# jordi-adell/mcarray

Hardware: AMD Instinct MI355X
Metric: STFT frames/sec, 8-mic GCC-PHAT + SRP-PHAT(361) + delay-and-sum beamform @48kHz/1024-pt (higher is better)
Workload: dtype f32 (SRP operands adaptive); 1 GPU; BASELINE configs[2] geometry (8-mic ULA 0.04 m, 48 kHz, N=1024, hop 512, 361 angles, 1 source, no power floor), 8 arrays x 4096 frames per GPU per step; channel rows padded by 64 floats; arrays_per_gpu=8, frames_per_array=4096, srp_precision=adaptive, parallelism=arrays sharded over 1 GPU(s), all_gather of DOA bins+prob

## Files before the change

### mcarray_amd/csrc/api.hip

```cpp
#include "../../include/mcarray_hip.h"
#include "fft1024c.h"
#include "kernels.h"
#include "knobs.h"
#include "stage.h"

#include <chrono>
#include <cmath>
#include <cstdio>
#include <cstdlib>
#include <cstring>
#include <string>
#include <thread>
#include <vector>

using namespace mca;

namespace {

std::string g_create_error;

struct TimedEvent { int id; hipEvent_t a, b; };

}

// ... 1521 lines not shown
static int ensure_bf_table(mca_hip_ctx *c)
{
    if (!c->d_bftab && c->n2048) {
        HIP_TRY(c, hipMalloc((void **)&c->d_bftab, (size_t)(c->D + 1) * c->M * 1032 * sizeof(float2)));
        c->bf_pairs = c->M;
        const double unit = (double)c->cfg.sample_rate / (double)c->N / 346.1;
        hipLaunchKernelGGL(k_bf_table_2048, dim3(c->D + 1, c->M), dim3(256), 0, nullptr, c->d_bftab, c->d_grid, c->d_micx, c->M, unit);
        HIP_TRY(c, hipGetLastError());
        HIP_TRY(c, hipDeviceSynchronize());
        return MCA_HIP_OK;
    }
    if (c->d_bftab || !wave_beamformer_applies(c)) return MCA_HIP_OK;
    const int np = (c->M + 1) / 2;
    HIP_TRY(c, hipMalloc((void **)&c->d_bftab, (size_t)(c->D + 1) * np * 1024 * sizeof(float2)));
    c->bf_pairs = np;
    const double unit = (double)c->cfg.sample_rate / (double)FFT_N / 346.1;
    hipLaunchKernelGGL(k_bf_table, dim3(c->D + 1, np), dim3(256), 0, nullptr, c->d_bftab, c->d_grid, c->d_micx, c->M, np, unit);
    HIP_TRY(c, hipGetLastError());
    HIP_TRY(c, hipDeviceSynchronize());
    return MCA_HIP_OK;
}

static int separate_impl(mca_hip_ctx *c, const float *pcm, long long array_stride, long long mic_stride,
                         int n_arrays, int n_frames, const float *doa_rad, float *out_pcm, hipStream_t st, const int *doa_bin = nullptr)
{
    const size_t a0 = (size_t)c->a0;
    if (doa_bin && c->d_bftab && c->n2048 && (reinterpret_cast<uintptr_t>(out_pcm) & 7) == 0) {
        BeamformWaveArgs wa{};
        wa.pcm = pcm; wa.array_stride = array_stride; wa.mic_stride = mic_stride;
        wa.M = c->M; wa.n_pairs = c->M; wa.n_frames = n_frames; wa.S = c->S;
        wa.ft = 16;
        for (int ft = 2; ft <= 64; ++ft)
            if ((long long)n_arrays * c->S * ((n_frames + 4 * ft - 2) / (4 * ft - 1)) <= 2LL * c->n_cu) { wa.ft = ft; break; }
        wa.window = c->d_window; wa.doa_bin = doa_bin; wa.table = c->d_bftab; wa.out = out_pcm;
        wa.tail_in = c->d_tail[c->tail_cur] + a0 * c->S * c->H; wa.tail_out = c->d_tail[c->tail_cur ^ 1] + a0 * c->S * c->H;
        const int wgs = (n_frames + 4 * wa.ft - 2) / (4 * wa.ft - 1);
        const size_t smem_w = (size_t)(F1K_TWORDS + 4 * F1K_SCRATCH + 4 * 512) * sizeof(float2);
        time_begin(c, MCA_HIP_K_BEAMFORM, st);
        hipLaunchKernelGGL(k_beamform_wave_2048, dim3(wgs, n_arrays, c->S), dim3(256), smem_w, st, wa);
        time_end(c, st);
        HIP_TRY(c, hipGetLastError());
        return MCA_HIP_OK;
    }
    if (doa_bin && c->d_bftab && wave_beamformer_applies(c)) {
        BeamformWaveArgs wa{};
        wa.pcm = pcm; wa.array_stride = array_stride; wa.mic_stride = mic_stride;
        wa.M = c->M; wa.n_pairs = c->bf_pairs; wa.n_frames = n_frames; wa.S = c->S;
        wa.window = c->d_window; wa.doa_bin = doa_bin; wa.table = c->d_bftab; wa.out = out_pcm;
        wa.tail_in = c->d_tail[c->tail_cur] + a0 * c->S * c->H; wa.tail_out = c->d_tail[c->tail_cur ^ 1] + a0 * c->S * c->H;
        if (c->S >= 2 && c->M <= 8) {
            wa.ft = 16;
            while (wa.ft > 2 && (long long)n_arrays * ((n_frames + wa.ft - 1) / wa.ft) < 2048) wa.ft >>= 1;
            const int runs = (n_frames + wa.ft - 1) / wa.ft;
            const size_t smem_ms = (size_t)(F1K_TWORDS + 4 * F1K_SCRATCH) * sizeof(float2) + (size_t)4 * c->S * FFT_H * sizeof(float);
            const dim3 gms((runs + 3) / 4, n_arrays);
            time_begin(c, MCA_HIP_K_BEAMFORM, st);
#define BFMS(NPT)                                                                                                                   \
            do {                                                                                                                    \
                if (smem_ms > 64 * 1024) {                                                                                          \
                    HIP_TRY(c, hipFuncSetAttribute(reinterpret_cast<const void *>(&k_beamform_wave_ms<NPT, false>), hipFuncAttributeMaxDynamicSharedMemorySize, (int)smem_ms)); \
                    HIP_TRY(c, hipFuncSetAttribute(reinterpret_cast<const void *>(&k_beamform_wave_ms<NPT, true>), hipFuncAttributeMaxDynamicSharedMemorySize, (int)smem_ms));  \
                }                                                                                                                   \
                if (c->M & 1) hipLaunchKernelGGL((k_beamform_wave_ms<NPT, true>), gms, dim3(256), smem_ms, st, wa);                 \
                else hipLaunchKernelGGL((k_beamform_wave_ms<NPT, false>), gms, dim3(256), smem_ms, st, wa);                         \
            } while (0)
            if (c->bf_pairs == 1) {
                if (smem_ms > 64 * 1024) HIP_TRY(c, hipFuncSetAttribute(reinterpret_cast<const void *>(&k_beamform_wave_ms<1, false>), hipFuncAttributeMaxDynamicSharedMemorySize, (int)smem_ms));
                hipLaunchKernelGGL((k_beamform_wave_ms<1, false>), gms, dim3(256), smem_ms, st, wa);
            }
            else if (c->bf_pairs == 2) BFMS(2);
            else if (c->bf_pairs == 3) BFMS(3);
            else BFMS(4);
#undef BFMS
            time_end(c, st);
            HIP_TRY(c, hipGetLastError());
            return MCA_HIP_OK;
        }
        wa.ft = 2;
        while (wa.ft < 256 && (long long)n_arrays * c->S * ((n_frames + 4 * wa.ft - 2) / (4 * wa.ft - 1)) > 512) ++wa.ft;
        const int wgs = (n_frames + 4 * wa.ft - 2) / (4 * wa.ft - 1);
        const size_t smem = (size_t)(F1K_TWORDS + 4 * F1K_SCRATCH) * sizeof(float2) + 4 * FFT_H * sizeof(float);
        dim3 gb(wgs, n_arrays, c->S);
        if (c->S == 1 && (wgs & 1) == 0 && wa.ft >= 8 && (long long)wgs * n_arrays > (long long)c->n_cu * 3 / 2 && (long long)wgs * n_arrays <= 2LL * c->n_cu) {
            wa.skew = (3 * wa.ft + 8) / 16;
            if (wa.skew >= wa.ft) wa.skew = 0;
            else gb = dim3(n_arrays, wgs, c->S);
        }
        time_begin(c, MCA_HIP_K_BEAMFORM, st);
        if (c->M & 1) hipLaunchKernelGGL(k_beamform_wave<true>, gb, dim3(256), smem, st, wa);
        else hipLaunchKernelGGL(k_beamform_wave<false>, gb, dim3(256), smem, st, wa);
        time_end(c, st);
        HIP_TRY(c, hipGetLastError());
        return MCA_HIP_OK;
    }
    BeamformArgs ba{};
    ba.pcm = pcm; ba.array_stride = array_stride; ba.mic_stride = mic_stride;
    ba.M = c->M; ba.Mpad = c->M; ba.S = c->S; ba.n_frames = n_frames; ba.fs = c->cfg.sample_rate;
    ba.ft = 64;
    long long want_wgs = 512;
    if (c->generic) {
        const size_t smem_g = (size_t)(c->M + c->S) * (c->H + 1) * sizeof(float2) + (size_t)c->S * c->H * sizeof(float);
        const long long per_cu = std::max<long long>(1, std::min<long long>((160 * 1024) / (long long)smem_g, 2048 / gen_threads(c, true)));
        want_wgs = 256 * per_cu;
    }
    while (ba.ft > BF_NB && (long long)n_arrays * ((n_frames + ba.ft - 1) / ba.ft) < want_wgs) ba.ft >>= 1;
    ba.window = c->d_window; ba.mic_x = c->d_micx; ba.doa_rad = doa_rad; ba.out = out_pcm;
    ba.tail_in = c->d_tail[c->tail_cur] + a0 * c->S * c->H; ba.tail_out = c->d_tail[c->tail_cur ^ 1] + a0 * c->S * c->H;
    ba.N = c->N; ba.logH = c->logH; ba.tw = c->d_tw;
    if (c->n512) {
        const size_t smem = ((size_t)2 * 8 * 258 + 8 * FFT_SCRATCH + TW_WIN + (size_t)2 * c->S * c->M * 41) * sizeof(float2) + (size_t)2 * c->S * sizeof(double);
        ba.ft = 64;
        const long long per_cu = smem <= 80 * 1024 ? 2 : 1;
        while (ba.ft > 4 && (long long)n_arrays * ((n_frames + ba.ft - 1) / ba.ft) < 256 * per_cu) ba.ft >>= 1;
        HIP_TRY(c, hipFuncSetAttribute(reinterpret_cast<const void *>(k_beamform_512), hipFuncAttributeMaxDynamicSharedMemorySize, (int)smem));
        time_begin(c, MCA_HIP_K_BEAMFORM, st);
        hipLaunchKernelGGL(k_beamform_512, dim3((n_frames + ba.ft - 1) / ba.ft, n_arrays), dim3(512), smem, st, ba);
        time_end(c, st);
        HIP_TRY(c, hipGetLastError());
        return MCA_HIP_OK;
    }
    if (c->generic) {
        auto smem_for = [&](int s_pass) {
            return (size_t)(c->M + s_pass) * (c->H + 1) * sizeof(float2) + (size_t)s_pass * c->H * sizeof(float) + (size_t)(ba.ft + 1) * s_pass * sizeof(double) + 8;
        };
        int s_pass = c->S;
        while (s_pass > 1 && smem_for(s_pass) > 160 * 1024) --s_pass;
        const size_t smem = smem_for(s_pass);
        if (smem > 160 * 1024) return fail(c, MCA_HIP_ERR_UNSUPPORTED, "fft_size x n_mics exceeds the 160 KiB LDS of a CU");
        if (smem > 64 * 1024)
            HIP_TRY(c, hipFuncSetAttribute(reinterpret_cast<const void *>(k_beamform_gen), hipFuncAttributeMaxDynamicSharedMemorySize, (int)smem));
        time_begin(c, MCA_HIP_K_BEAMFORM, st);
        ba.S_all = c->S;
        for (int s0 = 0; s0 < c->S; s0 += s_pass) {
            ba.s0 = s0; ba.S = std::min(s_pass, c->S - s0);
// ... 740 lines not shown
```

### mcarray_amd/csrc/fft1024c.h

```cpp
#pragma once
#include "fft512.h"

namespace mca {

constexpr int F1K_ROW = 18;
constexpr int F1K_SCRATCH = 64 * F1K_ROW;
constexpr int F1K_TWORDS = 64 * F1K_ROW;

__device__ __forceinline__ void f1k_table_init(float2 *tab, int tid, int nthreads)
{
    for (int e = tid; e < 1024; e += nthreads) tab[(e >> 4) * F1K_ROW + (e & 15)] = twiddle(((e >> 4) * (e & 15)) & 1023, 1024, false);
}

__device__ __forceinline__ float2 csub_jb(float2 a, float2 b)
{
    v2f av = to_v2f(a), bv = to_v2f(b), r;
    asm("v_pk_fma_f32 %0, %2, 1.0, %1 op_sel:[1,0,0] op_sel_hi:[0,0,1] neg_hi:[1,0,0]" : "=v"(r) : "v"(av), "v"(bv));
    return from_v2f(r);
}
__device__ __forceinline__ float2 cadd_jb(float2 a, float2 b)
{
    v2f av = to_v2f(a), bv = to_v2f(b), r;
    asm("v_pk_fma_f32 %0, %2, 1.0, %1 op_sel:[1,0,0] op_sel_hi:[0,0,1] neg_lo:[1,0,0]" : "=v"(r) : "v"(av), "v"(bv));
    return from_v2f(r);
}
__device__ __forceinline__ float2 cscale(float2 a, float s)
{
    v2f av = to_v2f(a), sv = {s, s}, r;
    asm("v_pk_mul_f32 %0, %1, %2" : "=v"(r) : "v"(av), "v"(sv));
    return from_v2f(r);
}
__device__ __forceinline__ float2 cmul_mj(float2 a)
{
    v2f av = to_v2f(a), one = {1.f, 1.f}, r;
    asm("v_pk_mul_f32 %0, %1, %2 op_sel:[1,0] op_sel_hi:[0,1] neg_hi:[1,0]" : "=v"(r) : "v"(av), "v"(one));
    return from_v2f(r);
}
__device__ __forceinline__ float2 cmul_pj(float2 a)
{
    v2f av = to_v2f(a), one = {1.f, 1.f}, r;
    asm("v_pk_mul_f32 %0, %1, %2 op_sel:[1,0] op_sel_hi:[0,1] neg_lo:[1,0]" : "=v"(r) : "v"(av), "v"(one));
    return from_v2f(r);
}

template <bool INV>
__device__ __forceinline__ void bfly4(float2 &a0, float2 &a1, float2 &a2, float2 &a3)
{
    const float2 t0 = cadd(a0, a2), t1 = csub(a0, a2), t2 = cadd(a1, a3), t3 = csub(a1, a3);
    a0 = cadd(t0, t2);
    a2 = csub(t0, t2);
    if (!INV) { a1 = csub_jb(t1, t3); a3 = cadd_jb(t1, t3); }
    else { a1 = cadd_jb(t1, t3); a3 = csub_jb(t1, t3); }
}

__device__ __forceinline__ constexpr int dr16(int p) { return (p >> 2) + 4 * (p & 3); }

template <bool INV>
__device__ __forceinline__ void fft16(float2 (&v)[16])
{
    constexpr float R = 0.70710678118654752440f, C1 = 0.92387953251128675613f, S1 = 0.38268343236508977173f;
#pragma unroll
    for (int j = 0; j < 4; ++j) bfly4<INV>(v[j], v[j + 4], v[j + 8], v[j + 12]);
    const float2 w1 = make_float2(C1, -S1), w3 = make_float2(S1, -C1), w9 = make_float2(-C1, S1);
    if (!INV) {
        v[5] = cmul(v[5], w1);  v[9] = cscale(csub_jb(v[9], v[9]), R);   v[13] = cmul(v[13], w3);
        v[6] = cscale(csub_jb(v[6], v[6]), R);  v[10] = cmul_mj(v[10]);   v[14] = cscale(cadd_jb(v[14], v[14]), -R);
        v[7] = cmul(v[7], w3);  v[11] = cscale(cadd_jb(v[11], v[11]), -R); v[15] = cmul(v[15], w9);
    } else {
        v[5] = cmulc(v[5], w1); v[9] = cscale(cadd_jb(v[9], v[9]), R);   v[13] = cmulc(v[13], w3);
        v[6] = cscale(cadd_jb(v[6], v[6]), R);  v[10] = cmul_pj(v[10]);   v[14] = cscale(csub_jb(v[14], v[14]), -R);
        v[7] = cmulc(v[7], w3); v[11] = cscale(csub_jb(v[11], v[11]), -R); v[15] = cmulc(v[15], w9);
    }
#pragma unroll
    for (int q = 0; q < 4; ++q) bfly4<INV>(v[4 * q], v[4 * q + 1], v[4 * q + 2], v[4 * q + 3]);
}

__device__ __forceinline__ void lds_read16_b128(float2 (&v)[16], const float2 *p)
{
    typedef float v4f __attribute__((ext_vector_type(4)));
    v4f a[8];
    asm volatile(
        "ds_read_b128 %0, %8\n\tds_read_b128 %1, %8 offset:16\n\tds_read_b128 %2, %8 offset:32\n\tds_read_b128 %3, %8 offset:48\n\t"
        "ds_read_b128 %4, %8 offset:64\n\tds_read_b128 %5, %8 offset:80\n\tds_read_b128 %6, %8 offset:96\n\tds_read_b128 %7, %8 offset:112\n\t"
        "s_waitcnt lgkmcnt(0)"
        : "=&v"(a[0]), "=&v"(a[1]), "=&v"(a[2]), "=&v"(a[3]), "=&v"(a[4]), "=&v"(a[5]), "=&v"(a[6]), "=&v"(a[7])
        : "v"((unsigned)(uintptr_t)p)
        : "memory");
#pragma unroll
    for (int i = 0; i < 8; ++i) { v[2 * i] = make_float2(a[i].x, a[i].y); v[2 * i + 1] = make_float2(a[i].z, a[i].w); }
}

__device__ __forceinline__ void swap_rows32(float &a, float &b)
{
    const auto r = __builtin_amdgcn_permlane32_swap(__float_as_uint(a), __float_as_uint(b), false, false);
    a = __uint_as_float(r[0]); b = __uint_as_float(r[1]);
}
__device__ __forceinline__ void swap_rows16(float &a, float &b)
{
    const auto r = __builtin_amdgcn_permlane16_swap(__float_as_uint(a), __float_as_uint(b), false, false);
    a = __uint_as_float(r[0]); b = __uint_as_float(r[1]);
}
__device__ __forceinline__ void transpose_rows4(float2 &x0, float2 &x1, float2 &x2, float2 &x3)
{
    swap_rows32(x0.x, x2.x); swap_rows32(x0.y, x2.y); swap_rows32(x1.x, x3.x); swap_rows32(x1.y, x3.y);
    swap_rows16(x0.x, x1.x); swap_rows16(x0.y, x1.y); swap_rows16(x2.x, x3.x); swap_rows16(x2.y, x3.y);
}

struct F1kNoMid { __device__ __forceinline__ void operator()() const {} };

struct F1kLane {
    float2 wb[4];
    float2 t1[16];
    __device__ __forceinline__ void init(int lane)
    {
#pragma unroll
        for (int q = 1; q < 4; ++q) wb[q] = twiddle(((lane & 15) * q) & 63, 64, false);
    }
    __device__ __forceinline__ void load_t1(const float2 *tab, int lane)
    {
#pragma unroll
        for (int q = 0; q < 16; ++q) t1[q] = tab[lane * 18 + q];
    }
};

template <bool INV, int OPT = 3, typename Mid = F1kNoMid>
__device__ __forceinline__ void fft1024c(float2 (&v)[16], float2 *buf, int lane, const float2 *tab, const F1kLane &lc, Mid mid = Mid(), int row = -1)
{
    constexpr bool SCHED = OPT & 2, T1REG = OPT & 4;
    float2 tw[16];
    if (!T1REG) {
        lds_read16_b128(tw, tab + lane * F1K_ROW);
        if (SCHED) __builtin_amdgcn_sched_barrier(0);
    }
    fft16<INV>(v);
#pragma unroll
    for (int p = 1; p < 16; ++p) {
        const float2 w = T1REG ? lc.t1[dr16(p)] : tw[dr16(p)];
        v[p] = INV ? cmulc(v[p], w) : cmul(v[p], w);
    }
#pragma unroll
    for (int q = 0; q < 4; ++q) transpose_rows4(v[4 * q], v[4 * q + 1], v[4 * q + 2], v[4 * q + 3]);
#pragma unroll
    for (int q = 0; q < 4; ++q) bfly4<INV>(v[4 * q], v[4 * q + 1], v[4 * q + 2], v[4 * q + 3]);
    float2 *wr = buf + (lane >> 4) * (4 * F1K_ROW) + (lane & 15);
#pragma unroll
    for (int q = 0; q < 4; ++q)
#pragma unroll
        for (int kb = 0; kb < 4; ++kb) {
            if (kb != 0) v[4 * q + kb] = INV ? cmulc(v[4 * q + kb], lc.wb[kb]) : cmul(v[4 * q + kb], lc.wb[kb]);
            wr[(q + 16 * kb) * F1K_ROW] = v[4 * q + kb];
        }
    wave_lds_fence();
    mid();
    if (SCHED) __builtin_amdgcn_sched_barrier(0);
    lds_read16_b128(v, buf + (row < 0 ? lane : row) * F1K_ROW);
    wave_lds_fence();
    fft16<INV>(v);
}

}
```

### mcarray_amd/csrc/fft512.h

```cpp
#pragma once
#include <hip/hip_runtime.h>

namespace mca {

constexpr int FFT_N = 1024;
constexpr int FFT_H = 512;
constexpr int FFT_K = 513;
constexpr int FFT_SCRATCH = 576;
constexpr int FFT_ROW = 72;

typedef float v2f __attribute__((ext_vector_type(2)));
__device__ __forceinline__ v2f to_v2f(float2 a) { v2f r = {a.x, a.y}; return r; }
__device__ __forceinline__ float2 from_v2f(v2f a) { return make_float2(a.x, a.y); }

__device__ __forceinline__ float2 cmul(float2 a, float2 b)
{
    v2f av = to_v2f(a), bv = to_v2f(b), t, r;
    asm("v_pk_mul_f32 %0, %1, %2 op_sel:[1,0] op_sel_hi:[1,1]" : "=v"(t) : "v"(av), "v"(bv));
    asm("v_pk_fma_f32 %0, %1, %2, %3 op_sel:[0,0,1] op_sel_hi:[0,1,0] neg_lo:[0,0,1]" : "=v"(r) : "v"(av), "v"(bv), "v"(t));
    return from_v2f(r);
}
__device__ __forceinline__ float2 cmulc(float2 a, float2 b)
{
    v2f av = to_v2f(a), bv = to_v2f(b), t, r;
    asm("v_pk_mul_f32 %0, %1, %2 op_sel:[1,0] op_sel_hi:[1,1]" : "=v"(t) : "v"(bv), "v"(av));
    asm("v_pk_fma_f32 %0, %1, %2, %3 op_sel:[0,0,1] op_sel_hi:[1,0,0] neg_hi:[0,0,1]" : "=v"(r) : "v"(av), "v"(bv), "v"(t));
    return from_v2f(r);
}
__device__ __forceinline__ float2 cmac(float2 acc, float2 a, float2 b)
{
    v2f av = to_v2f(a), bv = to_v2f(b), cv = to_v2f(acc), u, r;
    asm("v_pk_fma_f32 %0, %1, %2, %3 op_sel:[1,0,1] op_sel_hi:[1,1,0] neg_hi:[1,0,0]" : "=v"(u) : "v"(bv), "v"(av), "v"(cv));
    asm("v_pk_fma_f32 %0, %1, %2, %3 op_sel:[0,0,1] op_sel_hi:[1,0,0]" : "=v"(r) : "v"(av), "v"(bv), "v"(u));
    return from_v2f(r);
}
__device__ __forceinline__ float2 cmacc(float2 acc, float2 a, float2 b)
{
    v2f av = to_v2f(a), bv = to_v2f(b), cv = to_v2f(acc), u, r;
    asm("v_pk_fma_f32 %0, %1, %2, %3 op_sel:[1,0,1] op_sel_hi:[1,1,0] neg_lo:[1,0,0]" : "=v"(u) : "v"(bv), "v"(av), "v"(cv));
    asm("v_pk_fma_f32 %0, %1, %2, %3 op_sel:[0,0,1] op_sel_hi:[1,0,0]" : "=v"(r) : "v"(av), "v"(bv), "v"(u));
    return from_v2f(r);
}
__device__ __forceinline__ float2 cnmac(float2 acc, float2 a, float2 b)
{
    v2f av = to_v2f(a), bv = to_v2f(b), cv = to_v2f(acc), u, r;
    asm("v_pk_fma_f32 %0, %1, %2, %3 op_sel:[1,0,1] op_sel_hi:[1,1,0] neg_lo:[1,0,0]" : "=v"(u) : "v"(bv), "v"(av), "v"(cv));
    asm("v_pk_fma_f32 %0, %1, %2, %3 op_sel:[0,0,1] op_sel_hi:[1,0,0] neg_lo:[1,0,0] neg_hi:[1,0,0]" : "=v"(r) : "v"(av), "v"(bv), "v"(u));
    return from_v2f(r);
}
__device__ __forceinline__ float2 cnmacc(float2 acc, float2 a, float2 b)
{
    v2f av = to_v2f(a), bv = to_v2f(b), cv = to_v2f(acc), u, r;
    asm("v_pk_fma_f32 %0, %1, %2, %3 op_sel:[1,0,1] op_sel_hi:[1,1,0] neg_hi:[1,0,0]" : "=v"(u) : "v"(bv), "v"(av), "v"(cv));
    asm("v_pk_fma_f32 %0, %1, %2, %3 op_sel:[0,0,1] op_sel_hi:[1,0,0] neg_lo:[1,0,0] neg_hi:[1,0,0]" : "=v"(r) : "v"(av), "v"(bv), "v"(u));
    return from_v2f(r);
}
__device__ __forceinline__ float2 cadd(float2 a, float2 b) { return make_float2(a.x + b.x, a.y + b.y); }
__device__ __forceinline__ float2 csub(float2 a, float2 b) { return make_float2(a.x - b.x, a.y - b.y); }
__device__ __forceinline__ float2 cconj(float2 a) { return make_float2(a.x, -a.y); }

__device__ __forceinline__ float2 twiddle(int num, int den, bool inv)
{
    float s, c;
    sincospif(2.0f * (float)num / (float)den, &s, &c);
    return make_float2(c, inv ? s : -s);
}

template <bool INV>
__device__ __forceinline__ void fft8(float2 (&v)[8])
{
    constexpr float R = 0.70710678118654752440f;
#pragma unroll
    for (int r = 0; r < 4; ++r) {
        float2 a = cadd(v[r], v[r + 4]);
        float2 b = csub(v[r], v[r + 4]);
        v[r] = a;
        if (r == 0) v[r + 4] = b;
        else if (r == 1) v[r + 4] = INV ? make_float2((b.x - b.y) * R, (b.x + b.y) * R)
                                        : make_float2((b.x + b.y) * R, (b.y - b.x) * R);
        else if (r == 2) v[r + 4] = INV ? make_float2(-b.y, b.x) : make_float2(b.y, -b.x);
        else v[r + 4] = INV ? make_float2((-b.x - b.y) * R, (b.x - b.y) * R)
                            : make_float2((b.y - b.x) * R, (-b.x - b.y) * R);
    }
#pragma unroll
    for (int h = 0; h < 8; h += 4) {
        float2 a0 = cadd(v[h], v[h + 2]), b0 = csub(v[h], v[h + 2]);
        float2 a1 = cadd(v[h + 1], v[h + 3]), b1 = csub(v[h + 1], v[h + 3]);
        v[h] = a0; v[h + 1] = a1; v[h + 2] = b0;
        v[h + 3] = INV ? make_float2(-b1.y, b1.x) : make_float2(b1.y, -b1.x);
    }
#pragma unroll
    for (int h = 0; h < 8; h += 2) {
        float2 a = cadd(v[h], v[h + 1]), b = csub(v[h], v[h + 1]);
        v[h] = a; v[h + 1] = b;
    }
}

__device__ __forceinline__ constexpr int br3(int i) { return ((i & 1) << 2) | (i & 2) | ((i >> 2) & 1); }

constexpr int TW_T1 = 0, TW_T2 = 512, TW_TS = 576, TW_WIN = 832, TW_WORDS = 1344;

struct FftTw {
    const float2 *tab;
    __device__ __forceinline__ float2 t1(int q, int lane) const { return tab[TW_T1 + q * 64 + lane]; }
    __device__ __forceinline__ float2 t2(int s, int lane) const { return tab[TW_T2 + s * 8 + (lane & 7)]; }
    __device__ __forceinline__ float2 ts(int i, int lane) const { return tab[TW_TS + i * 64 + lane]; }
    __device__ __forceinline__ float2 win(int r, int lane) const { return tab[TW_WIN + r * 64 + lane]; }
};

__device__ __forceinline__ void fft_table_init(float2 *tab, const float *window, int tid, int nthreads)
{
    for (int e = tid; e < TW_WIN; e += nthreads) {
        float2 v;
        if (e < TW_T2) { const int q = e >> 6, l = e & 63; v = twiddle((l * q) & 511, 512, false); }
        else if (e < TW_TS) { const int s = (e - TW_T2) >> 3, l0 = (e - TW_T2) & 7; v = twiddle((l0 * s) & 63, 64, false); }
        else { const int i = (e - TW_TS) >> 6, l = (e - TW_TS) & 63; v = twiddle(l + 64 * i, 1024, false); }
        tab[e] = v;
    }
    if (window)
        for (int e = tid; e < 512; e += nthreads) {
            const float2 w = reinterpret_cast<const float2 *>(window)[e];
            tab[TW_WIN + e] = make_float2(0.5f * w.x, 0.5f * w.y);
        }
}

__device__ __forceinline__ void wave_lds_fence()
{
    __builtin_amdgcn_fence(__ATOMIC_RELEASE, "wavefront");
    __builtin_amdgcn_wave_barrier();
    __builtin_amdgcn_fence(__ATOMIC_ACQUIRE, "wavefront");
}

template <bool INV, bool AHEAD = false>
__device__ __forceinline__ void cfft512_regs(float2 (&v)[8], float2 *buf, int lane, const FftTw &tw)
{
    float2 twa[8];
    if (AHEAD) {
#pragma unroll
        for (int i = 1; i < 8; ++i) twa[i] = tw.t1(br3(i), lane);
    }
    fft8<INV>(v);
#pragma unroll
    for (int i = 0; i < 8; ++i) {
        const int q = br3(i);
        const float2 w = (q == 0) ? make_float2(1.f, 0.f) : (AHEAD ? twa[i] : tw.t1(q, lane));
        buf[q * FFT_ROW + lane] = (q == 0) ? v[i] : (INV ? cmulc(v[i], w) : cmul(v[i], w));
    }
    wave_lds_fence();
    const int qq = lane >> 3, l0 = lane & 7;
#pragma unroll
    for (int l1 = 0; l1 < 8; ++l1) v[l1] = buf[qq * FFT_ROW + l0 + 8 * l1];
    wave_lds_fence();
    float2 twb[8];
    if (AHEAD) {
#pragma unroll
        for (int i = 1; i < 8; ++i) twb[i] = tw.t2(br3(i), lane);
    }
    fft8<INV>(v);
#pragma unroll
    for (int i = 0; i < 8; ++i) {
        const int s = br3(i);
        const float2 w = (s == 0) ? make_float2(1.f, 0.f) : (AHEAD ? twb[i] : tw.t2(s, lane));
        buf[qq + 66 * l0 + 8 * s] = (s == 0) ? v[i] : (INV ? cmulc(v[i], w) : cmul(v[i], w));
    }
    wave_lds_fence();
#pragma unroll
    for (int j = 0; j < 8; ++j) v[j] = buf[lane + 66 * j];
    wave_lds_fence();
    fft8<INV>(v);
}

template <bool AHEAD = false>
__device__ __forceinline__ void rfft1024(float2 (&v)[8], float2 *buf, int lane, const FftTw &tw)
{
    cfft512_regs<false, AHEAD>(v, buf, lane, tw);
#pragma unroll
    for (int i = 0; i < 8; ++i)
        if (br3(i) >= 4) buf[lane + 64 * br3(i)] = v[i];
    wave_lds_fence();
    float2 xk[4], xp[4];
#pragma unroll
    for (int i = 0; i < 4; ++i) {
        const int k = lane + 64 * i;
        const float2 zk = v[br3(i)];
        float2 zp = buf[(512 - k) & 511];
        if (k == 0) zp = zk;
        const float2 a = make_float2(zk.x + zp.x, zk.y - zp.y);
        const float2 d = make_float2(zk.x - zp.x, zk.y + zp.y);
        const float2 b = make_float2(d.y, -d.x);
        const float2 wb = cmul(tw.ts(i, lane), b);
        xk[i] = cadd(a, wb);
        xp[i] = cconj(csub(a, wb));
    }
    const float2 z256 = v[br3(4)];
    wave_lds_fence();
#pragma unroll
    for (int i = 0; i < 4; ++i) {
        const int k = lane + 64 * i;
        buf[k] = xk[i];
        buf[512 - k] = xp[i];
    }
    if (lane == 0) {
        buf[256] = make_float2(2.f * z256.x, -2.f * z256.y);
    }
    wave_lds_fence();
}

__device__ __forceinline__ void irfft1024(float2 *buf, int lane, const FftTw &tw)
{
    float2 v[8], zp[4];
#pragma unroll
    for (int i = 0; i < 4; ++i) {
        const int k = lane + 64 * i;
        float2 xk = buf[k];
        float2 xp = buf[512 - k];
        if (k == 0) { xk.y = 0.f; xp.y = 0.f; }
        const float2 a = make_float2(xk.x + xp.x, xk.y - xp.y);
        const float2 d = make_float2(xk.x - xp.x, xk.y + xp.y);
        const float2 b = cmulc(d, tw.ts(i, lane));
        v[i] = make_float2(a.x - b.y, a.y + b.x);
        zp[i] = make_float2(a.x + b.y, -a.y + b.x);
    }
// ... 132 lines not shown
```

### mcarray_amd/csrc/kernels_wave.hip

```cpp
#include <type_traits>

#include "fft1024c.h"
#include "mca_internal.h"
#include "cand_unit.h"
#include "phat_pairs.h"
#include "pair_balance.h"

namespace mca {

__global__ __launch_bounds__(256) void k_bf_table(float2 *tab, const float *grid, const double *mic_x, int M, int n_pairs, double unit)
{
    const int d = blockIdx.x, pr = blockIdx.y;
    const double doa = d == 0 ? 0.0 : (double)grid[d - 1];
    const double cd = cos(doa + 1.57079632679489661923);
    const double sc = 1.0 / ((double)M * 1024.0);
    float2 *row = tab + ((long long)d * n_pairs + pr) * 1024;
    for (int k = threadIdx.x; k < 1024; k += 256) {
        const int kap = k <= 512 ? k : k - 1024;
        double pa[2] = {0.0, 0.0}, pb[2] = {0.0, 0.0};
        for (int e = 0; e < 2; ++e) {
            const int c = 2 * pr + e;
            if (c >= M) continue;
            double turns = (double)kap * (unit * mic_x[c] * cd);
            turns -= rint(turns);
            double sn, cs;
            sincospi(2.0 * turns, &sn, &cs);
            if (k == 512) sn = 0.0;
            (e == 0 ? pa : pb)[0] = cs; (e == 0 ? pa : pb)[1] = sn;
        }
        row[k] = make_float2((float)((pa[0] + pb[1]) * sc), (float)((pa[1] - pb[0]) * sc));
    }
}

__device__ __forceinline__ float2 win_lo(float a, float b, v2f w)
{
    v2f x = {a, b}, r;
    asm("v_pk_mul_f32 %0, %1, %2 op_sel:[0,0] op_sel_hi:[1,0]" : "=v"(r) : "v"(x), "v"(w));
    return from_v2f(r);
}
__device__ __forceinline__ float2 win_hi(float a, float b, v2f w)
{
    v2f x = {a, b}, r;
    asm("v_pk_mul_f32 %0, %2, %1 op_sel:[1,0] op_sel_hi:[1,1]" : "=v"(r) : "v"(x), "v"(w));
    return from_v2f(r);
}

template <bool ODD>
__global__ __launch_bounds__(256, 2) void k_beamform_wave(BeamformWaveArgs p)
{
    constexpr int FOPT = 7;
    extern __shared__ __attribute__((aligned(16))) unsigned char smem_raw[];
    float2 *tab = reinterpret_cast<float2 *>(smem_raw);
    const int tid = threadIdx.x, lane = tid & 63, wave = __builtin_amdgcn_readfirstlane(tid >> 6);
    float2 *buf = tab + F1K_TWORDS + wave * F1K_SCRATCH;
    float *xcarry = reinterpret_cast<float *>(tab + F1K_TWORDS + 4 * F1K_SCRATCH);
    f1k_table_init(tab, tid, 256);
    F1kLane lc;
    lc.init(lane);
    __syncthreads();
    lc.load_t1(tab, lane);

    const int a = p.skew ? blockIdx.x : blockIdx.y;
    const long long as = (long long)a * p.S + blockIdx.z;
    int w0 = (int)blockIdx.x * (4 * p.ft - 1), ft = p.ft;
    if (p.skew) {
        const int g = blockIdx.y, half = gridDim.y >> 1, hi = p.ft + p.skew, lo = p.ft - p.skew;
        ft = g < half ? hi : lo;
        w0 = g < half ? g * (4 * hi - 1) : half * (4 * hi - 1) + (g - half) * (4 * lo - 1);
    }
    const int t0 = wave == 0 ? w0 : w0 + wave * ft - 1;
    const int t1 = min(w0 + (wave + 1) * ft - 1, p.n_frames);
    const bool active = t0 < t1;
    const bool lead_in = wave == 0 && t0 > 0;
    const bool deferred = wave > 0;
    const int tfirst = lead_in ? t0 - 1 : t0;
    const int NP = p.n_pairs;
    float carry[8], first[8];
#pragma unroll
    for (int i = 0; i < 8; ++i) { carry[i] = 0.f; first[i] = 0.f; }

    if (active) {
        v2f win[8];
#pragma unroll
        for (int i = 0; i < 8; ++i) { win[i].x = p.window[lane + 128 * i]; win[i].y = p.window[lane + 128 * i + 64]; }
        if (t0 == 0) {
#pragma unroll
            for (int i = 0; i < 8; ++i) carry[i] = p.tail_in[as * FFT_H + lane + 64 * i];
        }
        const float *base = p.pcm + (long long)a * p.array_stride + lane;
        const int *bins = p.doa_bin + (long long)a * p.n_frames * p.S + blockIdx.z;
        float xa[16], xb[16];
        auto load_pair = [&](int t, int pr) {
            const float *pa = base + (long long)(2 * pr) * p.mic_stride + (long long)t * FFT_H;
            const float *pb = (ODD && pr == NP - 1) ? pa : pa + p.mic_stride;
#pragma unroll
            for (int i = 0; i < 16; ++i) { xa[i] = pa[64 * i]; xb[i] = pb[64 * i]; }
        };
        load_pair(tfirst, 0);

        float2 W[16];
#pragma unroll
        for (int i = 0; i < 16; ++i) W[i] = make_float2(0.f, 0.f);
        int t = tfirst, pr = 0;
        const float2 *trow = p.table + ((long long)(bins[(long long)t * p.S] + 1) * NP) * 1024 + lane;
        for (;;) {
            float2 z[16], T[16];
#pragma unroll
            for (int i = 0; i < 8; ++i) { z[2 * i] = win_lo(xa[2 * i], xb[2 * i], win[i]); z[2 * i + 1] = win_hi(xa[2 * i + 1], xb[2 * i + 1], win[i]); }
            if (ODD && pr == NP - 1) {
#pragma unroll
                for (int i = 0; i < 16; ++i) z[i].y = 0.f;
            }
            const bool last_pair = pr == NP - 1, last = last_pair && t + 1 >= t1;
            load_pair(last ? t : (last_pair ? t + 1 : t), last ? pr : (last_pair ? 0 : pr + 1));
            __builtin_amdgcn_sched_barrier(0);
            fft1024c<false, FOPT>(z, buf, lane, tab, lc, [&]() {
#pragma unroll
                for (int i = 0; i < 16; ++i) T[i] = trow[pr * 1024 + 64 * dr16(i)];
            });
#pragma unroll
            for (int i = 0; i < 16; ++i) W[i] = cmac(W[i], z[i], T[i]);
            if (last_pair) {
                float2 y[16];
#pragma unroll
                for (int i = 0; i < 16; ++i) y[i] = W[dr16(i)];
                fft1024c<true, FOPT>(y, buf, lane, tab, lc);
                if (t >= t0) {
                    if (deferred && t == t0) {
#pragma unroll
                        for (int i = 0; i < 8; ++i) first[i] = y[dr16(i)].x;
                    } else {
                        float *o = p.out + as * p.n_frames * FFT_H + (long long)t * FFT_H + lane;
#pragma unroll
                        for (int i = 0; i < 8; ++i) o[64 * i] = carry[i] + y[dr16(i)].x;
                    }
                }
#pragma unroll
                for (int i = 0; i < 8; ++i) carry[i] = y[dr16(i + 8)].x;
                if (last) break;
#pragma unroll
                for (int i = 0; i < 16; ++i) W[i] = make_float2(0.f, 0.f);
                ++t; pr = 0;
                trow = p.table + ((long long)(bins[(long long)t * p.S] + 1) * NP) * 1024 + lane;
            } else {
                ++pr;
            }
        }
        if (t1 == p.n_frames) {
#pragma unroll
            for (int i = 0; i < 8; ++i) p.tail_out[as * FFT_H + lane + 64 * i] = carry[i];
        }
    }
#pragma unroll
    for (int i = 0; i < 8; ++i) xcarry[wave * FFT_H + lane + 64 * i] = carry[i];
    __syncthreads();
    if (active && deferred) {
        float *o = p.out + as * p.n_frames * FFT_H + (long long)t0 * FFT_H + lane;
#pragma unroll
        for (int i = 0; i < 8; ++i) o[64 * i] = xcarry[(wave - 1) * FFT_H + lane + 64 * i] + first[i];
    }
}
template __global__ void k_beamform_wave<false>(BeamformWaveArgs);
template __global__ void k_beamform_wave<true>(BeamformWaveArgs);

template <int NPT, bool ODD>
__global__ __launch_bounds__(256, 2) void k_beamform_wave_ms(BeamformWaveArgs p)
{
    extern __shared__ __attribute__((aligned(16))) unsigned char smem_raw[];
    float2 *tab = reinterpret_cast<float2 *>(smem_raw);
    const int tid = threadIdx.x, lane = tid & 63, wave = __builtin_amdgcn_readfirstlane(tid >> 6);
    float2 *buf = tab + F1K_TWORDS + wave * F1K_SCRATCH;
    const int S = p.S;
    float *carry = reinterpret_cast<float *>(tab + F1K_TWORDS + 4 * F1K_SCRATCH) + wave * (S * FFT_H) + lane;
    f1k_table_init(tab, tid, 256);
    F1kLane lc;
    lc.init(lane);
    __syncthreads();

    const int a = blockIdx.y;
    const int t0 = ((int)blockIdx.x * 4 + wave) * p.ft, t1 = min(t0 + p.ft, p.n_frames);
    if (t0 >= t1) return;
    const int tfirst = t0 > 0 ? t0 - 1 : 0;
    v2f win[8];
#pragma unroll
    for (int i = 0; i < 8; ++i) { win[i].x = p.window[lane + 128 * i]; win[i].y = p.window[lane + 128 * i + 64]; }
    for (int s = 0; s < S; ++s) {
#pragma unroll
        for (int i = 0; i < 8; ++i) carry[s * FFT_H + 64 * i] = t0 == 0 ? p.tail_in[((long long)a * S + s) * FFT_H + lane + 64 * i] : 0.f;
    }
    const float *base = p.pcm + (long long)a * p.array_stride + lane;
    const int *bins = p.doa_bin + (long long)a * p.n_frames * S;
    float xa[16], xb[16];
    auto load_pair = [&](int t, int pr) {
        const float *pa = base + (long long)(2 * pr) * p.mic_stride + (long long)t * FFT_H;
        const float *pb = (ODD && pr == NPT - 1) ? pa : pa + p.mic_stride;
#pragma unroll
        for (int i = 0; i < 16; ++i) { xa[i] = pa[64 * i]; xb[i] = pb[64 * i]; }
    };
    auto row_of = [&](int t, int s) { return p.table + ((long long)(bins[(long long)t * S + s] + 1) * NPT) * 1024 + lane; };
    load_pair(tfirst, 0);
    for (int t = tfirst; t < t1; ++t) {
        float2 Z[NPT][16];
#pragma unroll
        for (int pr = 0; pr < NPT; ++pr) {
            float2 z[16];
#pragma unroll
            for (int i = 0; i < 8; ++i) { z[2 * i] = win_lo(xa[2 * i], xb[2 * i], win[i]); z[2 * i + 1] = win_hi(xa[2 * i + 1], xb[2 * i + 1], win[i]); }
            if (ODD && pr == NPT - 1) {
                float zero;
                asm("v_mov_b32 %0, 0" : "=v"(zero));
#pragma unroll
                for (int i = 0; i < 16; ++i) z[i].y = zero;
            }
            fft1024c<false, 3>(z, buf, lane, tab, lc, [&]() { if (pr + 1 < NPT) load_pair(t, pr + 1); });
#pragma unroll
            for (int i = 0; i < 16; ++i) Z[pr][i] = z[i];
        }
        float2 T[16];
        const float2 *trow = row_of(t, 0);
#pragma unroll
        for (int i = 0; i < 16; ++i) T[i] = trow[64 * dr16(i)];
        auto source = [&](int s, auto last_tag) {
            constexpr bool LAST = decltype(last_tag)::value;
            float2 W[16];
#pragma unroll
            for (int pr = 0; pr < NPT; ++pr) {
                __builtin_amdgcn_sched_barrier(0);
#pragma unroll
                for (int i = 0; i < 16; ++i) {
                    W[i] = pr == 0 ? cmul(Z[0][i], T[i]) : cmac(W[i], Z[pr][i], T[i]);
                    if (pr + 1 < NPT) T[i] = trow[(pr + 1) * 1024 + 64 * dr16(i)];
                }
            }
            float2 y[16];
#pragma unroll
            for (int i = 0; i < 16; ++i) y[i] = W[dr16(i)];
            if (LAST) {
                fft1024c<true, 3>(y, buf, lane, tab, lc, [&]() { load_pair(min(t + 1, t1 - 1), 0); });
            } else {
                fft1024c<true, 3>(y, buf, lane, tab, lc);
                trow = row_of(t, s + 1);
#pragma unroll
                for (int i = 0; i < 16; ++i) T[i] = trow[64 * dr16(i)];
            }
            float *cs = carry + s * FFT_H;
            if (t >= t0) {
                float *o = p.out + ((long long)a * S + s) * p.n_frames * FFT_H + (long long)t * FFT_H + lane;
#pragma unroll
                for (int i = 0; i < 8; ++i) o[64 * i] = cs[64 * i] + y[dr16(i)].x;
            }
#pragma unroll
            for (int i = 0; i < 8; ++i) cs[64 * i] = y[dr16(i + 8)].x;
        };
        for (int s = 0; s + 1 < S; ++s) source(s, std::false_type());
        source(S - 1, std::true_type());
    }
    if (t1 == p.n_frames) {
        for (int s = 0; s < S; ++s) {
#pragma unroll
            for (int i = 0; i < 8; ++i) p.tail_out[((long long)a * S + s) * FFT_H + lane + 64 * i] = carry[s * FFT_H + 64 * i];
        }
    }
}
template __global__ void k_beamform_wave_ms<1, false>(BeamformWaveArgs);
template __global__ void k_beamform_wave_ms<2, false>(BeamformWaveArgs); template __global__ void k_beamform_wave_ms<2, true>(BeamformWaveArgs);
template __global__ void k_beamform_wave_ms<3, false>(BeamformWaveArgs); template __global__ void k_beamform_wave_ms<3, true>(BeamformWaveArgs);
template __global__ void k_beamform_wave_ms<4, false>(BeamformWaveArgs); template __global__ void k_beamform_wave_ms<4, true>(BeamformWaveArgs);

template <bool NOPHAT = false>
__device__ __forceinline__ float2 whiten4(float2 z, float &pw, float thr = 4e-30f, float unit = 0.5f)
{
    v2f zv = to_v2f(z), sq, r;
    asm("v_pk_mul_f32 %0, %1, %1" : "=v"(sq) : "v"(zv));
    pw = sq.x + sq.y;
    const float s = NOPHAT ? unit : (pw > thr ? __builtin_amdgcn_rsqf(pw) : 0.f);
    v2f sv = {s, s};
    asm("v_pk_mul_f32 %0, %1, %2 op_sel_hi:[1,0]" : "=v"(r) : "v"(zv), "v"(sv));
    return from_v2f(r);
}

template <bool PL2>
__device__ __forceinline__ void store_a_wave(_Float16 *row, unsigned voff, int cidx, float2 v, int Kp)
{
    const float2_t vv = {v.x, v.y};
    const half2_t hi = __builtin_convertvector(vv, half2_t);
    char *b = reinterpret_cast<char *>(row + 2 * cidx);
    *reinterpret_cast<half2_t *>(b + voff) = hi;
    if (PL2) {
        const float2_t back = __builtin_convertvector(hi, float2_t);
        *reinterpret_cast<half2_t *>(reinterpret_cast<char *>(row + Kp + 2 * cidx) + voff) = __builtin_convertvector(vv - back, half2_t);
    }
}
template <bool PL2>
__device__ __forceinline__ void store_a_wave(float *row, unsigned voff, int cidx, float2 v, int)
{
    *reinterpret_cast<float2 *>(reinterpret_cast<char *>(row + 2 * cidx) + 2 * voff) = v;
}

__device__ __forceinline__ unsigned or3(unsigned a, unsigned b, unsigned c)
{
    unsigned r;
    asm("v_or3_b32 %0, %1, %2, %3" : "=v"(r) : "v"(a), "v"(b), "v"(c));
    return r;
}

typedef __attribute__((address_space(3))) float lds_float_t;

__device__ __forceinline__ float wave_sum64(float v)
{
    asm("s_nop 1\n\tv_add_f32_dpp %0, %0, %0 quad_perm:[1,0,3,2] row_mask:0xf bank_mask:0xf\n\t"
        "s_nop 1\n\tv_add_f32_dpp %0, %0, %0 quad_perm:[2,3,0,1] row_mask:0xf bank_mask:0xf\n\t"
        "s_nop 1\n\tv_add_f32_dpp %0, %0, %0 row_ror:4 row_mask:0xf bank_mask:0xf\n\t"
        "s_nop 1\n\tv_add_f32_dpp %0, %0, %0 row_ror:8 row_mask:0xf bank_mask:0xf\n\t"
// ... 470 lines not shown
```

Before: 48.36 million frames/s.

## Replace complex 1024-point inverse FFT with real-output split via 512-point FFT

The beamformer's overlap-add synthesis previously ran a full complex 1024-point inverse FFT and kept only the real part. It now packs the Hermitian spectrum into a 512-point complex inverse FFT using split twiddles stored in LDS, then unpacks even and odd samples as float2. The table scale is halved to match the new normalisation. The 512-point FFT gains a packed-math radix-8 variant and a mid-callback hook to overlap the next PCM load. This adds LDS twiddle space and changes the output and carry indexing layout, so correctness depends on the new interleaved layout matching everywhere.

```diff
diff --git a/mcarray_amd/csrc/api.hip b/mcarray_amd/csrc/api.hip
--- a/mcarray_amd/csrc/api.hip
+++ b/mcarray_amd/csrc/api.hip
@@ -1597,7 +1597,7 @@
             wa.ft = 16;
             while (wa.ft > 2 && (long long)n_arrays * ((n_frames + wa.ft - 1) / wa.ft) < 2048) wa.ft >>= 1;
             const int runs = (n_frames + wa.ft - 1) / wa.ft;
-            const size_t smem_ms = (size_t)(F1K_TWORDS + 4 * F1K_SCRATCH) * sizeof(float2) + (size_t)4 * c->S * FFT_H * sizeof(float);
+            const size_t smem_ms = (size_t)(F1K_TWORDS + F1K_TSWORDS + 4 * F1K_SCRATCH) * sizeof(float2) + (size_t)4 * c->S * FFT_H * sizeof(float);
             const dim3 gms((runs + 3) / 4, n_arrays);
             time_begin(c, MCA_HIP_K_BEAMFORM, st);
 #define BFMS(NPT)                                                                                                                   \
@@ -1624,7 +1624,7 @@
         wa.ft = 2;
         while (wa.ft < 256 && (long long)n_arrays * c->S * ((n_frames + 4 * wa.ft - 2) / (4 * wa.ft - 1)) > 512) ++wa.ft;
         const int wgs = (n_frames + 4 * wa.ft - 2) / (4 * wa.ft - 1);
-        const size_t smem = (size_t)(F1K_TWORDS + 4 * F1K_SCRATCH) * sizeof(float2) + 4 * FFT_H * sizeof(float);
+        const size_t smem = (size_t)(F1K_TWORDS + F1K_TSWORDS + 4 * F1K_SCRATCH) * sizeof(float2) + 4 * FFT_H * sizeof(float);
         dim3 gb(wgs, n_arrays, c->S);
         if (c->S == 1 && (wgs & 1) == 0 && wa.ft >= 8 && (long long)wgs * n_arrays > (long long)c->n_cu * 3 / 2 && (long long)wgs * n_arrays <= 2LL * c->n_cu) {
             wa.skew = (3 * wa.ft + 8) / 16;
diff --git a/mcarray_amd/csrc/fft1024c.h b/mcarray_amd/csrc/fft1024c.h
--- a/mcarray_amd/csrc/fft1024c.h
+++ b/mcarray_amd/csrc/fft1024c.h
@@ -12,24 +12,6 @@
     for (int e = tid; e < 1024; e += nthreads) tab[(e >> 4) * F1K_ROW + (e & 15)] = twiddle(((e >> 4) * (e & 15)) & 1023, 1024, false);
 }
 
-__device__ __forceinline__ float2 csub_jb(float2 a, float2 b)
-{
-    v2f av = to_v2f(a), bv = to_v2f(b), r;
-    asm("v_pk_fma_f32 %0, %2, 1.0, %1 op_sel:[1,0,0] op_sel_hi:[0,0,1] neg_hi:[1,0,0]" : "=v"(r) : "v"(av), "v"(bv));
-    return from_v2f(r);
-}
-__device__ __forceinline__ float2 cadd_jb(float2 a, float2 b)
-{
-    v2f av = to_v2f(a), bv = to_v2f(b), r;
-    asm("v_pk_fma_f32 %0, %2, 1.0, %1 op_sel:[1,0,0] op_sel_hi:[0,0,1] neg_lo:[1,0,0]" : "=v"(r) : "v"(av), "v"(bv));
-    return from_v2f(r);
-}
-__device__ __forceinline__ float2 cscale(float2 a, float s)
-{
-    v2f av = to_v2f(a), sv = {s, s}, r;
-    asm("v_pk_mul_f32 %0, %1, %2" : "=v"(r) : "v"(av), "v"(sv));
-    return from_v2f(r);
-}
 __device__ __forceinline__ float2 cmul_mj(float2 a)
 {
     v2f av = to_v2f(a), one = {1.f, 1.f}, r;
@@ -106,8 +88,6 @@
     swap_rows16(x0.x, x1.x); swap_rows16(x0.y, x1.y); swap_rows16(x2.x, x3.x); swap_rows16(x2.y, x3.y);
 }
 
-struct F1kNoMid { __device__ __forceinline__ void operator()() const {} };
-
 struct F1kLane {
     float2 wb[4];
     float2 t1[16];
@@ -158,4 +138,54 @@
     fft16<INV>(v);
 }
 
+constexpr int F1K_TSWORDS = 256;
+
+__device__ __forceinline__ void f1k_split_init(float2 *ts, int tid, int nthreads)
+{
+    for (int e = tid; e < F1K_TSWORDS; e += nthreads) ts[e] = twiddle(e, 1024, false);
 }
+
+template <bool REG>
+struct F1kTw512 {
+    const float2 *tab;
+    const F1kLane &lc;
+    __device__ __forceinline__ float2 t1(int q, int lane) const { return REG ? lc.t1[2 * q] : tab[lane * F1K_ROW + 2 * q]; }
+    __device__ __forceinline__ float2 t2(int s, int lane) const { return tab[(lane & 7) * (8 * F1K_ROW) + 2 * s]; }
+};
+
+template <typename TW, typename Mid = F1kNoMid>
+__device__ __forceinline__ void ifft1024c_re(const float2 (&W)[16], float2 (&v)[8], float2 *buf, int lane, const float2 *ts, const TW &tw,
+                                             Mid mid = Mid())
+{
+#pragma unroll
+    for (int p = 0; p < 16; ++p) {
+        const int s = dr16(p);
+        if (s == 0 || (s >= 4 && s <= 8) || s >= 12) buf[lane + 64 * s] = W[p];
+    }
+    wave_lds_fence();
+    float2 zp[4];
+#pragma unroll
+    for (int i = 0; i < 4; ++i) {
+        const int k = lane + 64 * i;
+        const float2 wk = W[dr16(i)], wh = W[dr16(i + 8)], wm = buf[(1024 - k) & 1023], wl = buf[512 - k];
+        const float2 yk = make_float2(wk.x + wm.x, wk.y - wm.y);
+        const float2 yp = make_float2(wl.x + wh.x, wl.y - wh.y);
+        const float2 a = make_float2(yk.x + yp.x, yk.y - yp.y);
+        const float2 d = make_float2(yk.x - yp.x, yk.y + yp.y);
+        const float2 b = cmulc(d, ts[64 * i + lane]);
+        v[i] = cadd_jb(a, b);
+        zp[i] = cconj_sub_jb(a, b);
+    }
+    const float2 w256 = W[dr16(4)], w768 = W[dr16(12)];
+    wave_lds_fence();
+#pragma unroll
+    for (int i = 0; i < 4; ++i) buf[512 - lane - 64 * i] = zp[i];
+    if (lane == 0) buf[256] = make_float2(2.f * (w256.x + w768.x), 2.f * (w768.y - w256.y));
+    wave_lds_fence();
+#pragma unroll
+    for (int r = 4; r < 8; ++r) v[r] = buf[lane + 64 * r];
+    wave_lds_fence();
+    cfft512_regs<true, false, true>(v, buf, lane, tw, mid);
+}
+
+}
diff --git a/mcarray_amd/csrc/fft512.h b/mcarray_amd/csrc/fft512.h
--- a/mcarray_amd/csrc/fft512.h
+++ b/mcarray_amd/csrc/fft512.h
@@ -58,6 +58,31 @@
 __device__ __forceinline__ float2 cadd(float2 a, float2 b) { return make_float2(a.x + b.x, a.y + b.y); }
 __device__ __forceinline__ float2 csub(float2 a, float2 b) { return make_float2(a.x - b.x, a.y - b.y); }
 __device__ __forceinline__ float2 cconj(float2 a) { return make_float2(a.x, -a.y); }
+
+__device__ __forceinline__ float2 csub_jb(float2 a, float2 b)
+{
+    v2f av = to_v2f(a), bv = to_v2f(b), r;
+    asm("v_pk_fma_f32 %0, %2, 1.0, %1 op_sel:[1,0,0] op_sel_hi:[0,0,1] neg_hi:[1,0,0]" : "=v"(r) : "v"(av), "v"(bv));
+    return from_v2f(r);
+}
+__device__ __forceinline__ float2 cadd_jb(float2 a, float2 b)
+{
+    v2f av = to_v2f(a), bv = to_v2f(b), r;
+    asm("v_pk_fma_f32 %0, %2, 1.0, %1 op_sel:[1,0,0] op_sel_hi:[0,0,1] neg_lo:[1,0,0]" : "=v"(r) : "v"(av), "v"(bv));
+    return from_v2f(r);
+}
+__device__ __forceinline__ float2 cscale(float2 a, float s)
+{
+    v2f av = to_v2f(a), sv = {s, s}, r;
+    asm("v_pk_mul_f32 %0, %1, %2" : "=v"(r) : "v"(av), "v"(sv));
+    return from_v2f(r);
+}
+__device__ __forceinline__ float2 cconj_sub_jb(float2 a, float2 b)
+{
+    v2f av = to_v2f(a), bv = to_v2f(b), r;
+    asm("v_pk_fma_f32 %0, %2, 1.0, %1 op_sel:[1,0,0] op_sel_hi:[0,0,1] neg_hi:[0,0,1]" : "=v"(r) : "v"(av), "v"(bv));
+    return from_v2f(r);
+}
 
 __device__ __forceinline__ float2 twiddle(int num, int den, bool inv)
 {
@@ -96,6 +121,24 @@
     }
 }
 
+template <bool INV>
+__device__ __forceinline__ void fft8_pk(float2 (&v)[8])
+{
+    constexpr float R = 0.70710678118654752440f;
+    float2 a[4], b[4];
+#pragma unroll
+    for (int r = 0; r < 4; ++r) { a[r] = cadd(v[r], v[r + 4]); b[r] = csub(v[r], v[r + 4]); }
+    b[1] = INV ? cscale(cadd_jb(b[1], b[1]), R) : cscale(csub_jb(b[1], b[1]), R);
+    b[3] = INV ? cscale(csub_jb(b[3], b[3]), -R) : cscale(cadd_jb(b[3], b[3]), -R);
+    const float2 x0 = cadd(a[0], a[2]), x2 = csub(a[0], a[2]), x1 = cadd(a[1], a[3]), x3 = csub(a[1], a[3]);
+    const float2 y0 = INV ? cadd_jb(b[0], b[2]) : csub_jb(b[0], b[2]), y2 = INV ? csub_jb(b[0], b[2]) : cadd_jb(b[0], b[2]);
+    const float2 y1 = cadd(b[1], b[3]), y3 = csub(b[1], b[3]);
+    v[0] = cadd(x0, x1); v[1] = csub(x0, x1);
+    v[2] = INV ? cadd_jb(x2, x3) : csub_jb(x2, x3); v[3] = INV ? csub_jb(x2, x3) : cadd_jb(x2, x3);
+    v[4] = cadd(y0, y1); v[5] = csub(y0, y1);
+    v[6] = INV ? cadd_jb(y2, y3) : csub_jb(y2, y3); v[7] = INV ? csub_jb(y2, y3) : cadd_jb(y2, y3);
+}
+
 __device__ __forceinline__ constexpr int br3(int i) { return ((i & 1) << 2) | (i & 2) | ((i >> 2) & 1); }
 
 constexpr int TW_T1 = 0, TW_T2 = 512, TW_TS = 576, TW_WIN = 832, TW_WORDS = 1344;
@@ -131,15 +174,16 @@
     __builtin_amdgcn_fence(__ATOMIC_ACQUIRE, "wavefront");
 }
 
-template <bool INV, bool AHEAD = false>
-__device__ __forceinline__ void cfft512_regs(float2 (&v)[8], float2 *buf, int lane, const FftTw &tw)
+struct F1kNoMid { __device__ __forceinline__ void operator()() const {} };
+template <bool INV, bool AHEAD = false, bool PK = false, typename TW = FftTw, typename Mid = F1kNoMid>
+__device__ __forceinline__ void cfft512_regs(float2 (&v)[8], float2 *buf, int lane, const TW &tw, Mid mid = Mid())
 {
     float2 twa[8];
     if (AHEAD) {
 #pragma unroll
         for (int i = 1; i < 8; ++i) twa[i] = tw.t1(br3(i), lane);
     }
-    fft8<INV>(v);
+    if (PK) fft8_pk<INV>(v); else fft8<INV>(v);
 #pragma unroll
     for (int i = 0; i < 8; ++i) {
         const int q = br3(i);
@@ -147,6 +191,7 @@
         buf[q * FFT_ROW + lane] = (q == 0) ? v[i] : (INV ? cmulc(v[i], w) : cmul(v[i], w));
     }
     wave_lds_fence();
+    mid();
     const int qq = lane >> 3, l0 = lane & 7;
 #pragma unroll
     for (int l1 = 0; l1 < 8; ++l1) v[l1] = buf[qq * FFT_ROW + l0 + 8 * l1];
@@ -156,7 +201,7 @@
 #pragma unroll
         for (int i = 1; i < 8; ++i) twb[i] = tw.t2(br3(i), lane);
     }
-    fft8<INV>(v);
+    if (PK) fft8_pk<INV>(v); else fft8<INV>(v);
 #pragma unroll
     for (int i = 0; i < 8; ++i) {
         const int s = br3(i);
@@ -167,7 +212,7 @@
 #pragma unroll
     for (int j = 0; j < 8; ++j) v[j] = buf[lane + 66 * j];
     wave_lds_fence();
-    fft8<INV>(v);
+    if (PK) fft8_pk<INV>(v); else fft8<INV>(v);
 }
 
 template <bool AHEAD = false>
diff --git a/mcarray_amd/csrc/kernels_wave.hip b/mcarray_amd/csrc/kernels_wave.hip
--- a/mcarray_amd/csrc/kernels_wave.hip
+++ b/mcarray_amd/csrc/kernels_wave.hip
@@ -13,7 +13,7 @@
     const int d = blockIdx.x, pr = blockIdx.y;
     const double doa = d == 0 ? 0.0 : (double)grid[d - 1];
     const double cd = cos(doa + 1.57079632679489661923);
-    const double sc = 1.0 / ((double)M * 1024.0);
+    const double sc = 1.0 / ((double)M * 2048.0);
     float2 *row = tab + ((long long)d * n_pairs + pr) * 1024;
     for (int k = threadIdx.x; k < 1024; k += 256) {
         const int kap = k <= 512 ? k : k - 1024;
@@ -52,13 +52,15 @@
     extern __shared__ __attribute__((aligned(16))) unsigned char smem_raw[];
     float2 *tab = reinterpret_cast<float2 *>(smem_raw);
     const int tid = threadIdx.x, lane = tid & 63, wave = __builtin_amdgcn_readfirstlane(tid >> 6);
-    float2 *buf = tab + F1K_TWORDS + wave * F1K_SCRATCH;
-    float *xcarry = reinterpret_cast<float *>(tab + F1K_TWORDS + 4 * F1K_SCRATCH);
+    float2 *tsw = tab + F1K_TWORDS, *buf = tsw + F1K_TSWORDS + wave * F1K_SCRATCH;
+    float *xcarry = reinterpret_cast<float *>(tsw + F1K_TSWORDS + 4 * F1K_SCRATCH);
     f1k_table_init(tab, tid, 256);
+    f1k_split_init(tsw, tid, 256);
     F1kLane lc;
     lc.init(lane);
     __syncthreads();
     lc.load_t1(tab, lane);
+    const F1kTw512<true> tw5{tab, lc};
 
     const int a = p.skew ? blockIdx.x : blockIdx.y;
     const long long as = (long long)a * p.S + blockIdx.z;
@@ -75,17 +77,18 @@
     const bool deferred = wave > 0;
     const int tfirst = lead_in ? t0 - 1 : t0;
     const int NP = p.n_pairs;
-    float carry[8], first[8];
-#pragma unroll
-    for (int i = 0; i < 8; ++i) { carry[i] = 0.f; first[i] = 0.f; }
+    float2 carry[4], first[4];
+#pragma unroll
+    for (int r = 0; r < 4; ++r) { carry[r] = make_float2(0.f, 0.f); first[r] = make_float2(0.f, 0.f); }
 
     if (active) {
         v2f win[8];
 #pragma unroll
         for (int i = 0; i < 8; ++i) { win[i].x = p.window[lane + 128 * i]; win[i].y = p.window[lane + 128 * i + 64]; }
         if (t0 == 0) {
-#pragma unroll
-            for (int i = 0; i < 8; ++i) carry[i] = p.tail_in[as * FFT_H + lane + 64 * i];
+            const float *ti = p.tail_in + as * FFT_H + 2 * lane;
+#pragma unroll
+            for (int r = 0; r < 4; ++r) carry[r] = make_float2(ti[128 * r], ti[128 * r + 1]);
         }
         const float *base = p.pcm + (long long)a * p.array_stride + lane;
         const int *bins = p.doa_bin + (long long)a * p.n_frames * p.S + blockIdx.z;
@@ -121,22 +124,20 @@
 #pragma unroll
             for (int i = 0; i < 16; ++i) W[i] = cmac(W[i], z[i], T[i]);
             if (last_pair) {
-                float2 y[16];
-#pragma unroll
-                for (int i = 0; i < 16; ++i) y[i] = W[dr16(i)];
-                fft1024c<true, FOPT>(y, buf, lane, tab, lc);
+                float2 y[8];
+                ifft1024c_re(W, y, buf, lane, tsw, tw5);
                 if (t >= t0) {
                     if (deferred && t == t0) {
 #pragma unroll
-                        for (int i = 0; i < 8; ++i) first[i] = y[dr16(i)].x;
+                        for (int r = 0; r < 4; ++r) first[r] = y[br3(r)];
                     } else {
-                        float *o = p.out + as * p.n_frames * FFT_H + (long long)t * FFT_H + lane;
-#pragma unroll
-                        for (int i = 0; i < 8; ++i) o[64 * i] = carry[i] + y[dr16(i)].x;
+                        float *o = p.out + as * p.n_frames * FFT_H + (long long)t * FFT_H + 2 * lane;
+#pragma unroll
+                        for (int r = 0; r < 4; ++r) { o[128 * r] = carry[r].x + y[br3(r)].x; o[128 * r + 1] = carry[r].y + y[br3(r)].y; }
                     }
                 }
 #pragma unroll
-                for (int i = 0; i < 8; ++i) carry[i] = y[dr16(i + 8)].x;
+                for (int r = 0; r < 4; ++r) carry[r] = y[br3(r + 4)];
                 if (last) break;
 #pragma unroll
                 for (int i = 0; i < 16; ++i) W[i] = make_float2(0.f, 0.f);
@@ -147,17 +148,19 @@
             }
         }
         if (t1 == p.n_frames) {
-#pragma unroll
-            for (int i = 0; i < 8; ++i) p.tail_out[as * FFT_H + lane + 64 * i] = carry[i];
-        }
-    }
-#pragma unroll
-    for (int i = 0; i < 8; ++i) xcarry[wave * FFT_H + lane + 64 * i] = carry[i];
+            float *to = p.tail_out + as * FFT_H + 2 * lane;
+#pragma unroll
+            for (int r = 0; r < 4; ++r) { to[128 * r] = carry[r].x; to[128 * r + 1] = carry[r].y; }
+        }
+    }
+#pragma unroll
+    for (int r = 0; r < 4; ++r) { xcarry[wave * FFT_H + 2 * lane + 128 * r] = carry[r].x; xcarry[wave * FFT_H + 2 * lane + 128 * r + 1] = carry[r].y; }
     __syncthreads();
     if (active && deferred) {
-        float *o = p.out + as * p.n_frames * FFT_H + (long long)t0 * FFT_H + lane;
-#pragma unroll
-        for (int i = 0; i < 8; ++i) o[64 * i] = xcarry[(wave - 1) * FFT_H + lane + 64 * i] + first[i];
+        float *o = p.out + as * p.n_frames * FFT_H + (long long)t0 * FFT_H + 2 * lane;
+        const float *xc = xcarry + (wave - 1) * FFT_H + 2 * lane;
+#pragma unroll
+        for (int r = 0; r < 4; ++r) { o[128 * r] = xc[128 * r] + first[r].x; o[128 * r + 1] = xc[128 * r + 1] + first[r].y; }
     }
 }
 template __global__ void k_beamform_wave<false>(BeamformWaveArgs);
@@ -169,13 +172,15 @@
     extern __shared__ __attribute__((aligned(16))) unsigned char smem_raw[];
     float2 *tab = reinterpret_cast<float2 *>(smem_raw);
     const int tid = threadIdx.x, lane = tid & 63, wave = __builtin_amdgcn_readfirstlane(tid >> 6);
-    float2 *buf = tab + F1K_TWORDS + wave * F1K_SCRATCH;
+    float2 *tsw = tab + F1K_TWORDS, *buf = tsw + F1K_TSWORDS + wave * F1K_SCRATCH;
     const int S = p.S;
-    float *carry = reinterpret_cast<float *>(tab + F1K_TWORDS + 4 * F1K_SCRATCH) + wave * (S * FFT_H) + lane;
+    float *carry = reinterpret_cast<float *>(tsw + F1K_TSWORDS + 4 * F1K_SCRATCH) + wave * (S * FFT_H) + 2 * lane;
     f1k_table_init(tab, tid, 256);
+    f1k_split_init(tsw, tid, 256);
     F1kLane lc;
     lc.init(lane);
     __syncthreads();
+    const F1kTw512<false> tw5{tab, lc};
 
     const int a = blockIdx.y;
     const int t0 = ((int)blockIdx.x * 4 + wave) * p.ft, t1 = min(t0 + p.ft, p.n_frames);
@@ -186,7 +191,7 @@
     for (int i = 0; i < 8; ++i) { win[i].x = p.window[lane + 128 * i]; win[i].y = p.window[lane + 128 * i + 64]; }
     for (int s = 0; s < S; ++s) {
 #pragma unroll
-        for (int i = 0; i < 8; ++i) carry[s * FFT_H + 64 * i] = t0 == 0 ? p.tail_in[((long long)a * S + s) * FFT_H + lane + 64 * i] : 0.f;
+        for (int i = 0; i < 8; ++i) carry[s * FFT_H + 128 * (i >> 1) + (i & 1)] = t0 == 0 ? p.tail_in[((long long)a * S + s) * FFT_H + 2 * lane + 128 * (i >> 1) + (i & 1)] : 0.f;
     }
     const float *base = p.pcm + (long long)a * p.array_stride + lane;
     const int *bins = p.doa_bin + (long long)a * p.n_frames * S;
@@ -232,25 +237,23 @@
                     if (pr + 1 < NPT) T[i] = trow[(pr + 1) * 1024 + 64 * dr16(i)];
                 }
             }
-            float2 y[16];
-#pragma unroll
-            for (int i = 0; i < 16; ++i) y[i] = W[dr16(i)];
+            float2 y[8];
             if (LAST) {
-                fft1024c<true, 3>(y, buf, lane, tab, lc, [&]() { load_pair(min(t + 1, t1 - 1), 0); });
+                ifft1024c_re(W, y, buf, lane, tsw, tw5, [&]() { load_pair(min(t + 1, t1 - 1), 0); });
             } else {
-                fft1024c<true, 3>(y, buf, lane, tab, lc);
+                ifft1024c_re(W, y, buf, lane, tsw, tw5);
                 trow = row_of(t, s + 1);
 #pragma unroll
                 for (int i = 0; i < 16; ++i) T[i] = trow[64 * dr16(i)];
             }
             float *cs = carry + s * FFT_H;
             if (t >= t0) {
-                float *o = p.out + ((long long)a * S + s) * p.n_frames * FFT_H + (long long)t * FFT_H + lane;
-#pragma unroll
-                for (int i = 0; i < 8; ++i) o[64 * i] = cs[64 * i] + y[dr16(i)].x;
-            }
-#pragma unroll
-            for (int i = 0; i < 8; ++i) cs[64 * i] = y[dr16(i + 8)].x;
+                float *o = p.out + ((long long)a * S + s) * p.n_frames * FFT_H + (long long)t * FFT_H + 2 * lane;
+#pragma unroll
+                for (int r = 0; r < 4; ++r) { o[128 * r] = cs[128 * r] + y[br3(r)].x; o[128 * r + 1] = cs[128 * r + 1] + y[br3(r)].y; }
+            }
+#pragma unroll
+            for (int r = 0; r < 4; ++r) { cs[128 * r] = y[br3(r + 4)].x; cs[128 * r + 1] = y[br3(r + 4)].y; }
         };
         for (int s = 0; s + 1 < S; ++s) source(s, std::false_type());
         source(S - 1, std::true_type());
@@ -258,7 +261,7 @@
     if (t1 == p.n_frames) {
         for (int s = 0; s < S; ++s) {
 #pragma unroll
-            for (int i = 0; i < 8; ++i) p.tail_out[((long long)a * S + s) * FFT_H + lane + 64 * i] = carry[s * FFT_H + 64 * i];
+            for (int i = 0; i < 8; ++i) p.tail_out[((long long)a * S + s) * FFT_H + 2 * lane + 128 * (i >> 1) + (i & 1)] = carry[s * FFT_H + 128 * (i >> 1) + (i & 1)];
         }
     }
 }
```

Result: no change. 48.50 million frames/s (median of 6 runs) (+0.3%).
